# ChicyChen/LOCO-Edit

Measured on AMD Instinct MI355X. Metric: edit-directions/sec (top-5 PMP-Jacobian SVD @256^2) + vT cos-sim vs ref, higher is better.
Workload: dtype bf16x3 (split-bf16 MFMA operands, fp32 accumulate + fp32 storage); 1 GPU; CelebA-HQ DDPM 256x256 top-5 local basis (l_eye-sized mask, L=2400), t=0.6T, 12 power iterations, one GPU; multi_gpu_form=single, probes_total=5, probes_per_gpu=5, kept=5, n_iter=12, mask_L=2400, weights=synthetic seed 0, streams=2

## Files before the change

loco-edit_amd/csrc/conv_bf16_kernel.h:

```cpp
#pragma once
#include "kernels.h"
#include <cstdlib>
#include <type_traits>

namespace loco {


typedef float f32x16 __attribute__((ext_vector_type(16)));
typedef float f32x4 __attribute__((ext_vector_type(4)));
typedef f32x4 f32x4_u __attribute__((aligned(4)));
typedef float f32x2 __attribute__((ext_vector_type(2)));
typedef f32x2 f32x2_u __attribute__((aligned(4)));
typedef __bf16 bf16x8 __attribute__((ext_vector_type(8)));
typedef _Float16 f16x8 __attribute__((ext_vector_type(8)));
typedef short s16x8 __attribute__((ext_vector_type(8)));

enum : int { PR_BF16X3 = 0, PR_F16 = 1 };

constexpr int BKC = 16;
constexpr bool LIVE_MASK = true;
constexpr bool EARLY_W = true;
constexpr int NDUMMY = 8;

__device__ __forceinline__ float sigmoidf2_(float y) { return __builtin_amdgcn_rcpf(1.0f + __expf(-y)); }

__device__ __forceinline__ int idiv_small(int n, int d) {
    int q = (int)((float)n * __builtin_amdgcn_rcpf((float)d));
    const int r = n - q * d;
    q += (r >= d) ? 1 : ((r < 0) ? -1 : 0);
    return q;
}
__device__ __forceinline__ void idivmod_small(int n, int d, int& q, int& r) { q = idiv_small(n, d); r = n - q * d; }

template <int PR>
__device__ __forceinline__ int rec_off(int p, int q) {
    if constexpr (PR == PR_F16) return p * 32 + ((q ^ ((p >> 3) & 1)) << 4);
    else return p * 64 + ((q ^ ((p >> 2) & 3)) << 4);
}
template <int PR> constexpr int halo_pitch() { return PR == PR_F16 ? 48 : 80; }
template <int PR> constexpr int rec_bytes() { return PR == PR_F16 ? 32 : 64; }
template <int PR>
__device__ __forceinline__ int hrec_off(int p, int q) { return p * halo_pitch<PR>() + (q << 4); }

template <int PR>
__device__ __forceinline__ void cvt2(float a, float b, unsigned& hi, unsigned& lo) {
    if constexpr (PR == PR_F16) {
        _Float16 ha = (_Float16)a, hb = (_Float16)b;
        hi = (unsigned)__builtin_bit_cast(unsigned short, ha) | ((unsigned)__builtin_bit_cast(unsigned short, hb) << 16);
        lo = 0;
    } else {
        typedef float f32x2_ __attribute__((ext_vector_type(2)));
        typedef __bf16 bf16x2_ __attribute__((ext_vector_type(2)));
        hi = __builtin_bit_cast(unsigned, __builtin_convertvector((f32x2_){a, b}, bf16x2_));
        const float ha = __builtin_bit_cast(float, hi << 16), hb = __builtin_bit_cast(float, hi & 0xffff0000u);
// ... 387 lines not shown
                                           (fmaf(xb[0], vb[0], xb[1] * vb[1]) + fmaf(xb[2], vb[2], xb[3] * vb[3]));
            }
        }
    }
    if (tan_st) {
        constexpr int STEPS = rs_steps(NV, 64), LEFT = NV >> STEPS;
        static_assert((NV & (NV - 1)) == 0, "row sums per lane");
        rs_reduce<NV, 1, 64>(av, lane);
        if (lane < (1 << STEPS)) {
            int base = 0;
#pragma unroll
            for (int sb = 0; sb < STEPS; ++sb) base += ((lane >> sb) & 1) * (NV >> (sb + 1));
            const int ntl = (a.Hout * a.Wout) / NT, ntile = 2 * ntl;
            float* const sp = a.st_part + (long)b * C * ntile * 2;
#pragma unroll
            for (int i = 0; i < LEFT; ++i) {
                const int idx = base + i, hq = idx >> 1;
                const int h = hq / NP, q = hq - h * NP;
                const int co = ch0 + h * 32 + q * RSTEP + row0;
                sp[((long)co * ntile + pa * ntl + tile_id) * 2 + (idx & 1)] = av[i];
            }
        }
    }
}

template <int PR, int TAPS, int WM, int WN, int TM, int TN, int MODE, int STG, int PHASE = 0>
__device__ __forceinline__ void conv_lowp_body(const ConvArgs& a, f32x16 (&acc)[TM][TN]) {
    constexpr int NTHR = WM * WN * 64;
    constexpr int HP = halo_pitch<PR>();
    constexpr int RB = rec_bytes<PR>();
    constexpr int NPC = RB / 16;
    constexpr int MT = WM * TM * 32;
    constexpr int NT = WN * TN * 32;
    constexpr bool POLY = (TAPS == 4 && STG == 0), PIN = (TAPS == 4 && STG == 1);
    static_assert(TAPS != 4 || POLY || PIN, "4-tap kernels: the two polyphase forms");
    static_assert(!PIN || (MODE == CM_NONE && PHASE == 0), "polyphase input form: raw");
    constexpr int KS = (TAPS == 9) ? 3 : (TAPS == 4 ? 2 : 1);
    constexpr int HK = (TAPS == 1) ? 1 : 3;
    constexpr int NTS = KS;
    constexpr int NROW = KS;
    static_assert(!POLY || (WM == 2 && TM == 2 && MODE == CM_NONE && PHASE == 0), "polyphase output form: 128 x 256 tile, raw vector staging");
    constexpr bool NEEDP = (MODE == CM_TAN_SILU || MODE == CM_COT_SILU);
    constexpr bool GEN = (STG == 1 || STG == 2);
    constexpr int NITEM = GEN ? (2 * max_halo(NT, TAPS, STG == 2) + NTHR - 1) / NTHR : 1;
    constexpr int WTOT = NTS * MT * NPC;
    constexpr int NWV = (WTOT + NTHR - 1) / NTHR;
    constexpr bool XPF = (TAPS == 9 && STG != 2);
    constexpr int NWB = XPF ? 3 : 2;
    constexpr bool DEEP1 = (TAPS == 1 && STG == 1 && !NEEDP);
    constexpr int DEEP_D = 4;

    extern __shared__ __attribute__((aligned(16))) unsigned char smem_b[];
#ifdef LOCO_DUAL_STAMP
#define LP_STAMP(i) do { if (threadIdx.x == 0 && PHASE == 0) reinterpret_cast<unsigned long long*>(a.partial)[blockIdx.x * 8 + (i)] = __builtin_amdgcn_s_memtime(); } while (0)
#else
#define LP_STAMP(i) do { } while (0)
#endif
    LP_STAMP(0);
    constexpr int WBYTES = NTS * MT * RB;
    unsigned char* const Wsb = smem_b;
    unsigned char* Hsb;
    unsigned char* Ws = smem_b;
    unsigned char* Hs = smem_b;

    const int tid = threadIdx.x;
    const int lane = tid & 63;
    const int wave = tid >> 6;
    const int l31 = lane & 31;
    const int khalf = lane >> 5;
    const int wm = wave / WN, wn = wave % WN;

    const int S = a.stride;
    const int TW = (TAPS == 1 && PHASE == 0 && a.stride == 1 && !a.upsample && !a.zins && (a.Wout & (a.Wout - 1)) == 0)
                       ? (a.Wout < NT ? a.Wout : NT) : (a.Wout < 32 ? a.Wout : 32);
    const int TH = NT / TW;
    const int tiles_x = a.Wout / TW;
    int tile_id, cot_id, zid;
    {
        const int ntile = (a.Hout * a.Wout) / NT, ncot = (a.Cout + MT - 1) / MT, Z = a.B * a.nsplit;
        const int NTC = ntile * ncot, L = blockIdx.x;
        int T = 0;
// ... 65 lines not shown
    const long in_plane = PIN ? 4L * a.Hin * a.Win : (long)a.Hin * a.Win;

    int ipos[NITEM], ioct[NITEM];
    unsigned ivoff[NITEM];
    bool ival[NITEM];
#pragma unroll
    for (int i = 0; i < NITEM; ++i) {
        int it = tid + i * NTHR;
        int oct, pos;
        idivmod_small(it, halo_sz, oct, pos);
        int off = -1;
        if (it < 2 * halo_sz) {
            int hy, hx;
            idivmod_small(pos, halo_w, hy, hx);
            int Y = oy0 * S - a.pad + hy, X = ox0 * S - a.pad + hx;
            if (Y >= 0 && Y < LH && X >= 0 && X < LW) {
                if (a.upsample) off = (Y >> 1) * a.Win + (X >> 1);
                else if (a.zins) off = ((Y | X) & 1) ? -1 : (Y >> 1) * a.Win + (X >> 1);
                else off = PIN ? 4 * Y * a.Win + 2 * X : Y * a.Win + X;
            }
        } else {
            pos = -1; oct = 0;
        }
        ipos[i] = pos; ioct[i] = oct;
        ival[i] = off >= 0;
        ivoff[i] = (unsigned)(oct * 8 * (int)in_plane + (off >= 0 ? off : 0));
    }

    const int nseg = (halo_w + 3) >> 2;
    int v_q4 = 0, v_pos0 = -1, v_voff = 0, v_cnt = 0;
    unsigned v_pm = 0;
    int v_rec[4] = {0, 0, 0, 0};
    unsigned v_goff = 0;
    if constexpr (!GEN) {
        const int per_q = halo_h * nseg;
        const int nsg4 = (nseg + 3) >> 2, nhy2 = (halo_h + 1) >> 1;
        bool have = false;
        int hy = 0, sg = 0;
        if (32 * nsg4 * nhy2 <= NTHR) {
            const int hi = tid >> 5;
            v_q4 = (tid >> 3) & 3;
            int hq_, hr_;
            idivmod_small(hi, nsg4, hq_, hr_);
            sg = hr_ * 4 + (tid & 3);
            hy = hq_ * 2 + ((tid >> 2) & 1);
            have = hi < nsg4 * nhy2 && sg < nseg && hy < halo_h;
            if (!have) v_q4 = 0;
        } else if (tid < 4 * per_q) {
            int rem;
            idivmod_small(tid, per_q, v_q4, rem);
            idivmod_small(rem, nseg, hy, sg);
            have = true;
        }
        if (have) {
            int Y = oy0 - a.pad + hy, X0 = ox0 - a.pad + 4 * sg;
            bool rowok = (Y >= 0 && Y < a.Hin);
            v_pos0 = hy * halo_w + 4 * sg;
            v_cnt = halo_w - 4 * sg < 4 ? halo_w - 4 * sg : 4;
            v_voff = rowok ? Y * a.Win + X0 : 0;
#pragma unroll
            for (int pxi = 0; pxi < 4; ++pxi)
                if (rowok && X0 + pxi >= 0 && X0 + pxi < a.Win && pxi < v_cnt) v_pm |= 1u << pxi;
        }
#pragma unroll
        for (int pxi = 0; pxi < 4; ++pxi)
            v_rec[pxi] = (v_pos0 >= 0 && pxi < v_cnt) ? v_pos0 + pxi : halo_sz + (tid & (NDUMMY - 1));
        v_goff = (unsigned)(((long)v_q4 * 4 * in_plane + v_voff + 16) * 4);
// ... 342 lines not shown
#elif defined(LOCO_WI_2MFMA)
            acc[i][j] = __builtin_amdgcn_mfma_f32_32x32x16_bf16(ah, bl, acc[i][j], 0, 0, 0);
            acc[i][j] = __builtin_amdgcn_mfma_f32_32x32x16_bf16(ah, bh, acc[i][j], 0, 0, 0);
            (void)al;
            return;
#endif
            acc[i][j] = __builtin_amdgcn_mfma_f32_32x32x16_bf16(al, bh, acc[i][j], 0, 0, 0);
            acc[i][j] = __builtin_amdgcn_mfma_f32_32x32x16_bf16(ah, bl, acc[i][j], 0, 0, 0);
            acc[i][j] = __builtin_amdgcn_mfma_f32_32x32x16_bf16(ah, bh, acc[i][j], 0, 0, 0);
        }
    };
    auto mma_frag_head = [&](const Frag& f) { mma_one(f, 0, 0); };
    auto mma_frag_tail = [&](const Frag& f) {
#pragma unroll
        for (int i = 0; i < TM; ++i)
#pragma unroll
            for (int j = 0; j < TN; ++j)
                if (i + j > 0) mma_one(f, i, j);
    };

    const int nch = cend - cbeg;
    const int clast = cend - 1;
    auto cclamp = [&](int c) { return __builtin_amdgcn_readfirstlane(c < clast ? c : clast); };
    auto vres = [&](int x) -> int {
        if (x <= clast) { pf_live = true; return __builtin_amdgcn_readfirstlane(x); }
        pf_live = !LIVE_MASK;
        return clast;
    };
    auto stage_end = [&]() {
        asm volatile("s_waitcnt lgkmcnt(0)" ::: "memory");
        __builtin_amdgcn_s_barrier();
        asm volatile("" ::: "memory");
    };
    if constexpr (XPF) {
        Frag fr[2];
        auto stage_of = [&](int ci_, int row_, int& c_out, int& r_out) {
            c_out = cclamp(cbeg + ci_ + row_ / NROW);
            r_out = row_ % NROW;
        };
        LP_STAMP(1);
        if (nch > 0) {
            if constexpr (!(PHASE != 2 && EARLY_W)) {
                int c1, r1;
                dma_w(cbeg, 0, Wsb);
                stage_of(0, 1, c1, r1);
                dma_w(c1, r1, Wsb + WBYTES);
            }
            Hs = Hsb;
            if constexpr (!GEN && NPART == 2) {
                HaloRegs hr2;
                prefetch_hv(hr, cbeg, 0);
                prefetch_hv(hr2, cbeg, 1);
                stage_hv(hr, 0);
                stage_hv(hr2, 1);
            } else {
                prefetch_h(cbeg, 0);
                stage_h(cbeg, 0);
            }
            asm volatile("s_waitcnt vmcnt(0)" ::: "memory");
            prefetch_h(cclamp(cbeg + 1), 0);
            stage_end();
            Ws = Wsb; Hs = Hsb;
            load_frag(fr[0], 0, 0);
        }
        LP_STAMP(2);
        auto chunk_body = [&](auto ptag, const int ci) {
            constexpr int P = decltype(ptag)::value;
// ... 222 lines not shown
constexpr int lowp_min_waves(int taps, int nthr) { return (taps == 1 && nthr <= 256) ? 2 : 1; }
template <int TAPS, int WM, int WN, int TM, int TN, int MODE, int STG>
__global__ __launch_bounds__(WM * WN * 64, lowp_min_waves(TAPS, WM * WN * 64)) void conv_mfma_bf16x3(ConvArgs a) {
    f32x16 acc[TM][TN];
    conv_lowp_body<PR_BF16X3, TAPS, WM, WN, TM, TN, MODE, STG>(a, acc);
}
template <int TAPS, int WM, int WN, int TM, int TN, int MODE, int STG>
__global__ __launch_bounds__(WM * WN * 64, lowp_min_waves(TAPS, WM * WN * 64)) void conv_mfma_f16(ConvArgs a) {
    f32x16 acc[TM][TN];
    conv_lowp_body<PR_F16, TAPS, WM, WN, TM, TN, MODE, STG>(a, acc);
}

template <int PR, int WM, int WN, int TM, int TN, int MODE>
__device__ __forceinline__ void conv_lowp_kcat(const ConvArgs& a) {
    f32x16 acc[TM][TN];
    conv_lowp_body<PR, 9, WM, WN, TM, TN, MODE, 0, 1>(a, acc);
    ConvArgs a2 = a;
    a2.in = a.in2; a2.in_bs = a.in2_bs; a2.Cin = a.Cin2; a2.wb = a.wb2; a2.mode = CM_NONE; a2.pad = 0; a2.in_padded = a.in2_padded;
    conv_lowp_body<PR, 1, WM, WN, TM, TN, CM_NONE, 1, 2>(a2, acc);
}
template <int WM, int WN, int TM, int TN, int MODE>
__global__ __launch_bounds__(WM * WN * 64) void conv_kcat_bf16x3(ConvArgs a) { conv_lowp_kcat<PR_BF16X3, WM, WN, TM, TN, MODE>(a); }
template <int WM, int WN, int TM, int TN, int MODE>
__global__ __launch_bounds__(WM * WN * 64) void conv_kcat_f16(ConvArgs a) { conv_lowp_kcat<PR_F16, WM, WN, TM, TN, MODE>(a); }

template <int PR, int TAPS, int WM, int WN, int TM, int TN, int MODE, int STG>
static void launch_one_b2(const ConvArgs& a, hipStream_t st) {
    constexpr int MT = WM * TM * 32, NT = WN * TN * 32;
    constexpr int KS = (TAPS == 9) ? 3 : (TAPS == 4 ? 2 : 1), HK = (TAPS == 1) ? 1 : 3;
    int TW = a.Wout < 32 ? a.Wout : 32;
    int TH = NT / TW;
    int halo_w = (TW - 1) * a.stride + HK, halo_h = (TH - 1) * a.stride + HK;
    const int nwb = (TAPS == 9 && STG != 2) ? 3 : 2;
    size_t lds = (size_t)nwb * KS * MT * rec_bytes<PR>() + 2 * ((size_t)halo_w * halo_h + NDUMMY) * halo_pitch<PR>();
    const size_t stage_bytes = (size_t)WM * 32 * NT * 4;
    if (lds < stage_bytes) lds = stage_bytes;
    dim3 grid(((a.Hout * a.Wout) / NT) * ((a.Cout + MT - 1) / MT) * a.B * a.nsplit);
    void (*kern)(ConvArgs);
    if constexpr (PR == PR_F16) kern = &conv_mfma_f16<TAPS, WM, WN, TM, TN, MODE, STG>;
    else kern = &conv_mfma_bf16x3<TAPS, WM, WN, TM, TN, MODE, STG>;
    if (lds > 64 * 1024) {
        static DeviceOnce once;
        if (first_on_device(once)) {
            (void)hipFuncSetAttribute(reinterpret_cast<const void*>(kern), hipFuncAttributeMaxDynamicSharedMemorySize,
                                      160 * 1024);
        }
    }
    hipLaunchKernelGGL(kern, grid, dim3(WM * WN * 64), lds, st, a);
}

template <int PR, int TAPS, int WM, int WN, int TM, int TN, int MODE>
static void launch_one_b(const ConvArgs& a, hipStream_t st) {
    const bool general = a.stride != 1 || a.upsample || a.zins || (a.Cin % BKC) != 0 || !a.in_padded;
    if constexpr (MODE == CM_NONE) {
        if (a.stride == 2) launch_one_b2<PR, TAPS, WM, WN, TM, TN, MODE, 2>(a, st);
        else if (TAPS == 9 && !general) launch_one_b2<PR, TAPS, WM, WN, TM, TN, MODE, 0>(a, st);
        else launch_one_b2<PR, TAPS, WM, WN, TM, TN, MODE, 1>(a, st);
        return;
    }
    if constexpr (MODE == CM_GN_SILU || MODE == CM_TAN_SILU || MODE == CM_GN_GELU) {
        if (general) { launch_one_b2<PR, TAPS, WM, WN, TM, TN, MODE, 1>(a, st); return; }
    }
    launch_one_b2<PR, TAPS, WM, WN, TM, TN, MODE, 0>(a, st);
}


template <int PR, int MODE>
void launch_kcat_b(const ConvArgs& a, hipStream_t st) {
    constexpr int WM = 2, WN = 4, TM = 2, TN = 2, MT = 128, NT = 256;
    const int TW = a.Wout < 32 ? a.Wout : 32, TH = NT / TW;
    size_t lds = (size_t)3 * 3 * MT * rec_bytes<PR>() + 2 * ((size_t)(TW + 2) * (TH + 2) + NDUMMY) * halo_pitch<PR>();
    dim3 grid(((a.Hout * a.Wout) / NT) * ((a.Cout + MT - 1) / MT) * a.B * a.nsplit);
    void (*kern)(ConvArgs);
    if constexpr (PR == PR_F16) kern = &conv_kcat_f16<WM, WN, TM, TN, MODE>;
    else kern = &conv_kcat_bf16x3<WM, WN, TM, TN, MODE>;
    static DeviceOnce once;
    if (first_on_device(once))
        (void)hipFuncSetAttribute(reinterpret_cast<const void*>(kern), hipFuncAttributeMaxDynamicSharedMemorySize, 160 * 1024);
    hipLaunchKernelGGL(kern, grid, dim3(WM * WN * 64), lds, st, a);
}

template <int PR>
void launch_poly_b(const ConvArgs& a, hipStream_t st) {
    ConvArgs v = a;
    v.Cout = 4 * a.Cout; v.Hout = a.Hin; v.Wout = a.Win;
    v.upsample = 0; v.zins = 0; v.stride = 1; v.pad = 1; v.nsplit = 1;
    launch_one_b2<PR, 4, 2, 4, 2, 2, CM_NONE, 0>(v, st);
}

template <int PR>
void launch_poly_in_b(const ConvArgs& a, hipStream_t st) {
    ConvArgs v = a;
    v.Cin = 4 * a.Cin; v.Hin = a.Hin / 2; v.Win = a.Win / 2;
    v.upsample = 0; v.zins = 0; v.stride = 1; v.pad = 1; v.nsplit = 1;
    launch_one_b2<PR, 4, 2, 4, 2, 2, CM_NONE, 1>(v, st);
}

template <int PR, int TAPS, int MODE>
void launch_tile_b(const ConvArgs& a, hipStream_t st) {
    switch (a.tile) {
        case 5:
            launch_one_b<PR, TAPS, 2, 4, 2, 2, MODE>(a, st);
            break;
        case 0: launch_one_b<PR, TAPS, 2, 2, 2, 2, MODE>(a, st); break;
        case 1: launch_one_b<PR, TAPS, 4, 1, 1, 2, MODE>(a, st); break;
        case 2: launch_one_b<PR, TAPS, 1, 4, 1, 1, MODE>(a, st); break;
        default: launch_one_b<PR, TAPS, 2, 2, 1, 1, MODE>(a, st); break;
    }
}


}
```

loco-edit_amd/csrc/conv_plan.hip:

```cpp
#include "kernels.h"
#include <cstdio>
#include <cstdlib>

namespace loco {

constexpr int BKC = 16;
constexpr int BKF = 8;

static const int kMT[6] = {128, 128, 32, 64, 128, 128}, kNT[6] = {128, 64, 128, 64, 256, 256};

static int env_int(const char* name, int dflt) {
    const char* e = getenv(name);
    return e ? atoi(e) : dflt;
}
static int pick_tile(int Cout, int HW) {
    if (HW >= 128) return Cout > 32 ? 0 : 2;
    return Cout > 64 ? 1 : 3;
}

static int conv_pick_nsplit(int Cin, int Cout, int Hout, int Wout, int B) {
    const int t = pick_tile(Cout, Hout * Wout);
    long blocks = (long)((Hout * Wout) / kNT[t]) * ((Cout + kMT[t] - 1) / kMT[t]) * B;
    int nchunks = (Cin + BKF - 1) / BKF;
    if (blocks >= 384 || nchunks < 8) return 1;
// ... 15 lines not shown
}

constexpr int kTile0MaxHW = 65536;

static int bf16_tile_of(const ConvArgs& a, int tile_override = -1) {
    int tile = conv_bf16_pick_tile(a.Cout, a.Hout * a.Wout, a.B, tile_override);
    if (tile == 4) tile = 5;
    if (tile == 5 && a.taps == 1 && !a.gemm && a.B >= 2 && a.Hout * a.Wout <= kTile0MaxHW) return 0;
    if (a.stride == 2 && tile == 5) tile = 0;
    return tile;
}
static int tile_for(const ConvArgs& a, int prec, int tile_override) {
    return prec ? bf16_tile_of(a, tile_override) : pick_tile(a.Cout, a.Hout * a.Wout);
}
static int conv_bf16_tile_pixels(const ConvArgs& a) { return a.poly == 1 ? 512 : a.gemm ? 256 : kNT[a.tile]; }
int conv_bf16_tile_couts(const ConvArgs& a) { return a.gemm ? 64 * a.gemm_tm : kMT[a.tile]; }

static bool conv_poly_ok(const ConvEnv& e, const ConvArgs& a, int taps) {
    static const bool on = env_int("LOCO_POLYPHASE", 1) != 0;
    if (!on || e.prec < 1 || taps != 9 || a.mode != CM_NONE || !(a.upsample || a.zins) || a.stride != 1) return false;
    if (!(e.prec == 2 ? a.wph : a.wpb) || !a.in_padded || a.res || a.Cin2 > 0 || a.cot_d) return false;
    if (a.upsample ? a.pad != 1 : (a.pad != 1 && a.pad != 2)) return false;
    if ((a.Cin % BKC) != 0 || (a.Cout % 128) != 0 || a.B < 2) return false;
    if (a.Hin * a.Win < 4096 || a.Win < 32 || (a.Win % 32) != 0 || (a.Hin % 8) != 0) return false;
    return a.Hout == 2 * a.Hin && a.Wout == 2 * a.Win;
}
static bool conv_poly_in_ok(const ConvEnv& e, const ConvArgs& a, int taps) {
    static const bool on = env_int("LOCO_POLYPHASE", 1) != 0;
    if (!on || e.prec < 1 || taps != 9 || a.mode != CM_NONE || !a.pool2 || a.upsample || a.zins || a.stride != 1 || a.pad != 1) return false;
    if (!(e.prec == 2 ? a.wqh : a.wqb) || a.res || a.bias2 || a.Cin2 > 0 || a.cot_d) return false;
    if ((a.Cin % BKC) != 0 || (a.Cout % 128) != 0 || a.B < 2 || ((a.Hin | a.Win) & 1)) return false;
    if (a.Hout * a.Wout < 4096 || a.Wout < 32 || (a.Wout % 32) != 0 || (a.Hout % 8) != 0) return false;
    return a.Hin == 2 * a.Hout && a.Win == 2 * a.Wout;
}

static int conv_bf16_pick_nsplit(int Cin, int Cout, int Hout, int Wout, int B, int chip_share, int taps, int lanes) {
    const int HW = Hout * Wout;
    int t = conv_bf16_pick_tile(Cout, HW, B, -1);
    if (t == 4) t = 5;
    if (taps == 1 && t == 5 && B >= 2 && HW <= kTile0MaxHW) t = 0;
    long blocks = (long)(HW / kNT[t]) * ((Cout + kMT[t] - 1) / kMT[t]) * B;
    int nchunks = (Cin + BKC - 1) / BKC;
    int target = chip_share > 1 ? 256 / chip_share : (lanes == 2 ? 240 : 256);
    if (target < 32) target = 32;
    if (blocks >= target / 2 || nchunks < 8) return 1;
    int want = (int)(target / blocks);
    int maxs = nchunks / 4;
    if (want > maxs) want = maxs;
    if (want > 32) want = 32;
    return want < 1 ? 1 : want;
}

static bool conv_lowp_can_kcat(const ConvArgs& a) {
    static const bool on = env_int("LOCO_KCAT", 1) != 0;
    return on && a.Cin2 > 0 && a.nsplit == 1 && bf16_tile_of(a) == 5 && a.stride == 1 && !a.upsample && !a.zins && a.pad == 1 &&
           (a.Cin % BKC) == 0 && (a.Cin2 % BKC) == 0 && a.in_padded &&
           (a.mode == CM_GN_SILU || a.mode == CM_GN_GELU || a.mode == CM_TAN_SILU);
}
static bool conv_lowp_can_fuse_stats(const ConvArgs& a) {
    return a.nsplit <= 1 && !a.gemm && (a.Cout % conv_bf16_tile_couts(a)) == 0;
}

static bool conv_pair_ok(const ConvArgs& a) {
    static const bool on = env_int("LOCO_CONV_PAIR", 1) != 0;
    if (!on || a.poly || a.Hout * a.Wout < 16384 || a.taps != 9 || a.Cin2 > 0 || a.nsplit != 1 || a.stride != 1 || a.upsample || a.zins ||
        a.pad != 1 || !a.in_padded || (a.Cin % (2 * BKC)) != 0 || (a.Cout % 128) != 0 || (a.Wout % 32) != 0 || (a.Hout % 8) != 0)
// ... 92 lines not shown
        return epi;
    }
    const bool cot_cache = q->kind == ST_COT && q->norm && q->sx && x.poly != 1;
    if ((q->kind == ST_TAN || cot_cache) && e.fuse_lin && !x.cot_d && conv_lowp_can_fuse_stats(x)) {
        const size_t lane_off = (size_t)e.lane_s0 * (q->keep_floats / e.max_batch);
        const bool keptl = q->kind == ST_TAN && q->keep && s0 == 0 && x.B == B && lane_off + need <= q->keep_floats;
        if (keptl || (q->norm && need <= e.stpart_floats)) {
            x.st_part = keptl ? q->keep + lane_off : e.stpart; x.st_kind = q->kind; x.st_x = q->prim;
            if (q->kind == ST_COT) x.st_sx = q->sx;
            if (keptl) *keep_ntile = ntile;
            return epi;
        }
    }
    return alone;
}

static ConvLaunch plan_launch(const ConvEnv& e, const StatAsk* q, bool want, const ConvArgs& x, int s0, int B, int* keep_ntile) {
    ConvLaunch l;
    l.args = x;
    l.s0 = s0;
    l.args.tile = tile_for(x, e.prec, -1);
    l.stats = stats_route(e, q, want, l.args, s0, B, keep_ntile);
    if (l.stats == SR_EPI || l.stats == SR_KEEP) l.ntile = (x.Hout * x.Wout) / conv_bf16_tile_pixels(l.args);
    conv_plan_tile_pair(l.args, e.prec, -1);
    return l;
}

ConvPlan plan_conv(const ConvEnv& e, const ConvArgs& a0, int taps, const StatAsk* q, const ConvArgs* sc) {
    ConvPlan p;
    ConvArgs a = a0;
    a.taps = taps;
    a.gemm = 0;
    a.poly = 0;
    if (a.pool2) {
        if (conv_poly_in_ok(e, a, taps)) a.poly = 2;
        else {
            p.pool_after = true; p.pool_out = a.out; p.pool_out_bs = a.out_bs; p.pool_acc = a.accumulate;
            a.out = a.pool_tmp; a.out_bs = a.pool_tmp_bs; a.Hout = a.Hin; a.Wout = a.Win; a.accumulate = 0; a.pool2 = 0;
        }
    }
    if (sc) {
        ConvArgs t = a;
        t.nsplit = e.prec >= 1 ? conv_bf16_pick_nsplit(a.Cin, a.Cout, a.Hout, a.Wout, a.B, e.chip_share, 9, e.lanes) : 2;
        t.in2 = sc->in; t.in2_bs = sc->in_bs; t.Cin2 = sc->Cin;
        const long per_probe = (long)((a.Hout * a.Wout) / 256) * ((a.Cout + 127) / 128);
        if (e.prec >= 1 && taps == 9 && !short_tail(per_probe, a.B) && !a.bias2 && conv_lowp_can_kcat(t)) {
            a.in2 = sc->in; a.in2_bs = sc->in_bs; a.Cin2 = sc->Cin; a.in2_padded = sc->in_padded;
            a.wb2 = e.prec == 2 ? sc->wh : sc->wb;
            a.bias2 = sc->bias; a.bias2_bs = 0;
            a.res = nullptr;
        } else {
            p.sc_first = true;
            a.res = sc->out; a.res_bs = sc->out_bs;
        }
    }
    if (e.prec == 2) a.wb = a.wh;
    a.no_deep = e.deep1 ? 0 : 1;
    a.nsplit = e.prec >= 1 ? conv_bf16_pick_nsplit(a.Cin, a.Cout, a.Hout, a.Wout, a.B, e.chip_share, taps, e.lanes)
                           : conv_pick_nsplit(a.Cin, a.Cout, a.Hout, a.Wout, a.B);
    if (a.cot_d) {
        ConvArgs t = a;
        t.tile = bf16_tile_of(t);
        const long per_probe = (long)((a.Hout * a.Wout) / conv_bf16_tile_pixels(t)) * ((a.Cout + 127) / 128);
        p.cot = e.prec >= 1 && taps == 1 && a.nsplit == 1 && !short_tail(per_probe, a.B) && conv_lowp_can_fuse_stats(t);
        if (!p.cot) { a.cot_d = nullptr; a.cot_d_bs = 0; a.cot_sx = nullptr; a.cot_tc = nullptr; a.cot_tc_bs = 0; }
    }
    while (a.nsplit > 1 && (size_t)a.nsplit * a.B * a.Cout * a.Hout * a.Wout > e.partial_floats) a.nsplit >>= 1;
    if (a.nsplit < 1) a.nsplit = 1;
// ... 99 lines not shown
```

loco-edit_amd/csrc/engine_diag.hip:

```cpp
#include <cmath>
#include <cstdio>
#include <cstdlib>
#include <cstring>
#include <initializer_list>

#include "../../include/loco_hip_diag.h"
#include "conv_plan_text.h"
#include "engine_internal.h"

using namespace loco;
using namespace loco::eng;

static void release_since(loco_ctx* c, hipStream_t st, size_t owned0, size_t bytes0) {
    (void)hipStreamSynchronize(st);
    while (c->owned.size() > owned0) { (void)hipFree(c->owned.back()); c->owned.pop_back(); }
    c->bytes = bytes0;
}

__global__ void diag_fill_records(unsigned char* rec, long nrec, int wpitch, unsigned seed, float scale) {
    const long r = (long)blockIdx.x * 256 + threadIdx.x;
    if (r >= nrec) return;
    const int idx = (int)(r % wpitch);
    unsigned short hi[16], lo[16];
    for (int k = 0; k < 16; ++k) {
// ... 49 lines not shown
    a.prim = c->arenaP; a.prim_bs = 0; a.sx = c->sxcache;
    a.w = wf; a.wb = wf; a.wh = wf;
    a.out = out; a.out_bs = out_e; a.Cout = cout; a.Hout = H; a.Wout = W; a.B = B;
    a.mode = mode; a.pad = taps == 9 ? 1 : 0; a.in_padded = 1; a.taps = taps;
    if (geom == 4) {
        a.pool2 = 1; a.pool_tmp = out; a.pool_tmp_bs = out_e;
        a.out = out + out_e * B; a.out_bs = out_e / 4; a.Hout = H / 2; a.Wout = W / 2;
        a.wqb = wf; a.wqh = wf;
    } else if (geom) {
        a.Hin = H / 2; a.Win = W / 2;
        if (geom == 1) a.upsample = 1; else { a.zins = 1; a.pad = geom == 2 ? 2 : 1; }
        a.wpb = wf; a.wph = wf;
    }
    a.sc = c->statsP; a.sh = c->statsP + cin; a.scsh_bs = 0; a.mr = c->statsP + 2 * cin; a.mr_bs = 0;
    a.gamma_ = c->statsP; a.tst = c->statsT; a.tst_bs = c->prog->stats_per_sample; a.cpg = cin / c->cfg.gn_groups;
    a.tc = c->statsT + 64; a.tc_bs = c->prog->stats_per_sample;
    if (a.cpg < 1) a.cpg = 1;
    a.nsplit = 1; a.partial = c->partial;
    a.partial_floats = c->partial_floats - wfl * 2;
    if (getenv("LOCO_BENCH_COT") && atoi(getenv("LOCO_BENCH_COT")) && taps == 1) {
        if ((in_e + 2 * out_e) * B > (long)c->cfg.max_batch * c->prog->per_sample || out_e > c->prog->sx_total ||
            2L * cout > c->prog->stats_per_sample) { c->err = "bench_conv: cot operands exceed the arenas"; return -2; }
        launch_fill_random(out + out_e * B, out_e * B, 8u, zs, st);
        if (out_e > in_e) launch_fill_random(reinterpret_cast<float*>(c->sxcache), 2 * out_e, 3u, zs, st);
        a.cot_d = out + out_e * B; a.cot_d_bs = out_e; a.cot_sx = c->sxcache; a.cot_tc = c->statsT; a.cot_tc_bs = c->prog->stats_per_sample;
    }
    if (getenv("LOCO_BENCH_ACC") && atoi(getenv("LOCO_BENCH_ACC"))) a.accumulate = 1;
    conv_plan_family(a, c->prec);
    if (const char* e = getenv("LOCO_DUAL_WHATIF")) a.no_deep = atoi(e);
    conv_plan_tile_pair(a, c->prec, tile);
    if (geom) {
        ConvEnv e;
        e.prec = c->prec; e.partial = a.partial; e.partial_floats = a.partial_floats; e.max_batch = c->cfg.max_batch;
        a.poly = plan_conv(e, a, taps, nullptr, nullptr).l[0].args.poly;
        if (a.poly) a.nsplit = 1;
        if (geom == 4 && a.poly != 2) { c->err = "bench_conv: the shape does not take the pooled polyphase launch"; return -2; }
    }
    auto run = [&]() {
        if (c->prec == 1) launch_conv_bf16x3(a, taps, st);
        else if (c->prec == 2) launch_conv_f16(a, taps, st);
        else launch_conv(a, taps, st);
        launch_conv_splitk_reduce(a, st);
    };
    run();
    HIPCHK(c, hipEventRecord(c->ev0, st));
    for (int i = 0; i < iters; ++i) run();
    HIPCHK(c, hipEventRecord(c->ev1, st));
    HIPCHK(c, hipEventSynchronize(c->ev1));
    c->bench_out = out; c->bench_out_count = (int64_t)out_e * B;
    float ms = 0.f;
    HIPCHK(c, hipEventElapsedTime(&ms, c->ev0, c->ev1));
    *ms_avg = ms / iters;
    HIPCHK(c, hipGetLastError());
    return 0;
}

}
__global__ void diag_scale_tc(const float* tc, const float* mr, int C, int cpg, long n, int by_rstd, float* out) {
    const long i = (long)blockIdx.x * 256 + threadIdx.x;
    if (i >= n) return;
    const float f = by_rstd ? mr[2 * (int)((i % C) / cpg) + 1] : 1.0f;
    out[2 * i] = f * tc[2 * i];
    out[2 * i + 1] = f * tc[2 * i + 1];
}
extern "C" {
int loco_debug_conv(loco_ctx* c, const loco_conv_desc* d, char* plan, int64_t cap, void* stream) {
    if (!c) return -2;
// ... 619 lines not shown
```

loco-edit_amd/csrc/kernels.h:

```cpp
#pragma once
#include <hip/hip_runtime.h>
#include <stdint.h>

namespace loco {

struct DeviceOnce { bool seen[64] = {}; };
inline bool first_on_device(DeviceOnce& f) {
    int d = 0;
    (void)hipGetDevice(&d);
    d &= 63;
    if (f.seen[d]) return false;
    f.seen[d] = true;
    return true;
}


enum ConvMode : int {
    CM_NONE = 0,
    CM_GN_SILU = 1,
    CM_GN = 2,
    CM_TAN_SILU = 3,
    CM_COT_SILU = 4,
    CM_GN_GELU = 5,
};
// ... 23 lines not shown
    const float* res; long res_bs;
    const float* sc; const float* sh; long scsh_bs;
    const float* mr; long mr_bs;
    const float* gamma_;
    const float* tst; long tst_bs;
    const float* tc; long tc_bs;
    int cpg;
    int mode;
    int stride;
    int pad;
    int upsample;
    int zins;
    int in_padded;
    int accumulate;
    int nsplit;
    int taps;
    int no_deep;
    float* partial;
    int B;
    float* st_part; int st_kind;
    const float* st_x; const float2* st_sx;
    const float* in2; long in2_bs; int Cin2; int in2_padded;
    const void* wb2;
    const float* cot_d; long cot_d_bs; const float2* cot_sx; const float* cot_tc; long cot_tc_bs;
    int act;
    float res_scale;
    int gemm, gemm_tm;
    size_t partial_floats;
    int tile, pair;
    const void* wpb; const void* wph;
    int poly;
    int pool2; float* pool_tmp; long pool_tmp_bs;
    const void* wqb; const void* wqh;
};

enum PolyKind : int { POLY_UP = 0, POLY_ZINS_PAD2 = 1, POLY_ZINS_PAD1 = 2 };
inline int polyphase_vcout(int C, int a, int b, int co) { return ((a * (C / 64) + co / 64) * 2 + b) * 64 + (co % 64); }
void polyphase_fold(int kind, int nin, int nout, const float* w, long so, long si, long st, float* out);
void polyphase_fold_in(int nin, int nout, const float* w, long so, long si, long st, float* out, int noutP);

void launch_conv(const ConvArgs& a, int taps, hipStream_t st);
void launch_conv_bf16x3(const ConvArgs& a, int taps, hipStream_t st);
void launch_conv_f16(const ConvArgs& a, int taps, hipStream_t st);
void launch_conv_splitk_reduce(const ConvArgs& a, hipStream_t st);

struct ConvEnv {
    int prec = 1;
    int chip_share = 1;
    int lanes = 1, lane_s0 = 0;
    float* partial = nullptr; size_t partial_floats = 0;
    float* stpart = nullptr; size_t stpart_floats = 0;
    bool fuse_stats = true, fuse_lin = true, deep1 = true;
    int max_batch = 1;
};

struct StatAsk {
    int kind = ST_NONE;
    bool norm = false;
    const float2* sx = nullptr;
    const float* prim = nullptr;
    float* keep = nullptr; size_t keep_floats = 0;
};

enum StatRoute : int {
    SR_NONE = 0,
    SR_EPI = 1,
// ... 220 lines not shown
```

Measured before the change: 20.65 edit-directions/s.

## Add row-staged vectorized polyphase input conv path with deeper halo buffering

Adds a new staging form (STG==3) for the pooled polyphase-input 4-tap conv. Each thread loads contiguous float4 runs of the padded full-resolution input, covering two row parities, and splits them into bf16 hi/lo halo records for both column phases. It uses four halo buffers so the next channel pair's halo stores overlap the current MMAs. The aim is fewer scattered gather loads and better overlap of loads with compute. In exchange it uses more LDS, which may cut occupancy, and it only runs when the input is padded.

```diff
diff --git a/loco-edit_amd/csrc/conv_bf16_kernel.h b/loco-edit_amd/csrc/conv_bf16_kernel.h
--- a/loco-edit_amd/csrc/conv_bf16_kernel.h
+++ b/loco-edit_amd/csrc/conv_bf16_kernel.h
@@ -1,5 +1,6 @@
 #pragma once
 #include "kernels.h"
+#include "poly_in_vec.h"
 #include <cstdlib>
 #include <type_traits>
 
@@ -20,6 +21,11 @@
 constexpr int BKC = 16;
 constexpr bool LIVE_MASK = true;
 constexpr bool EARLY_W = true;
+#ifndef LOCO_PIV_NHB
+#define LOCO_PIV_NHB 4
+#endif
+constexpr int PIV_NHB = LOCO_PIV_NHB;
+static_assert(PIV_NHB == 4 || PIV_NHB == 2, "halo buffers of the row-staged polyphase input form");
 constexpr int NDUMMY = 8;
 
 __device__ __forceinline__ float sigmoidf2_(float y) { return __builtin_amdgcn_rcpf(1.0f + __expf(-y)); }
@@ -473,7 +479,7 @@
     constexpr int NPC = RB / 16;
     constexpr int MT = WM * TM * 32;
     constexpr int NT = WN * TN * 32;
-    constexpr bool POLY = (TAPS == 4 && STG == 0), PIN = (TAPS == 4 && STG == 1);
+    constexpr bool POLY = (TAPS == 4 && STG == 0), PIN = (TAPS == 4 && (STG == 1 || STG == 3)), PINV = (TAPS == 4 && STG == 3);
     static_assert(TAPS != 4 || POLY || PIN, "4-tap kernels: the two polyphase forms");
     static_assert(!PIN || (MODE == CM_NONE && PHASE == 0), "polyphase input form: raw");
     constexpr int KS = (TAPS == 9) ? 3 : (TAPS == 4 ? 2 : 1);
@@ -488,6 +494,7 @@
     constexpr int NWV = (WTOT + NTHR - 1) / NTHR;
     constexpr bool XPF = (TAPS == 9 && STG != 2);
     constexpr int NWB = XPF ? 3 : 2;
+    constexpr int NHB = PINV ? PIV_NHB : 2;
     constexpr bool DEEP1 = (TAPS == 1 && STG == 1 && !NEEDP);
     constexpr int DEEP_D = 4;
 
@@ -619,7 +626,7 @@
     unsigned v_pm = 0;
     int v_rec[4] = {0, 0, 0, 0};
     unsigned v_goff = 0;
-    if constexpr (!GEN) {
+    if constexpr (!GEN && !PINV) {
         const int per_q = halo_h * nseg;
         const int nsg4 = (nseg + 3) >> 2, nhy2 = (halo_h + 1) >> 1;
         bool have = false;
@@ -1028,7 +1035,93 @@
         __builtin_amdgcn_s_barrier();
         asm volatile("" ::: "memory");
     };
-    if constexpr (XPF) {
+    if constexpr (PINV) {
+        const int cpp = a.Cin >> 6;
+        const int npair = 2 * cpp;
+        const int H2 = 2 * a.Hin, W2 = 2 * a.Win;
+        const bool have = tid < PIV_ITEMS;
+        const PolyInVecItem it0 = poly_in_vec_item(have ? tid : 0, oy0, ox0, 0, H2, W2);
+        const PolyInVecItem it1 = poly_in_vec_item(have ? tid : 0, oy0, ox0, 1, H2, W2);
+        const int p_oct = have ? it0.oct : ((tid >> 3) & 1);
+        const unsigned obase = have ? (unsigned)(it0.oct * 8) * (unsigned)in_plane : 0u;
+        const unsigned gob0 = (obase + (have ? it0.goff : 0u)) * 4u, gob1 = (obase + (have ? it1.goff : 0u)) * 4u;
+        const bool gin0 = have && it0.inside, gin1 = have && it1.inside;
+        int p_rec[2];
+#pragma unroll
+        for (int h = 0; h < 2; ++h) p_rec[h] = (have && it0.rec[h] >= 0) ? it0.rec[h] : halo_sz + (tid & (NDUMMY - 1));
+        f32x4 dq[8];
+        const long pb4 = in_plane * 4;
+        auto wchunk = [&](int pi, int q) { return __builtin_amdgcn_readfirstlane(poly_in_vec_wchunk(pi, q, cpp)); };
+        auto piv_load = [&](int pi) {
+            const bool live = LIVE_MASK ? (pi < npair) : true;
+            const int pc = pi < npair ? pi : npair - 1;
+            const int p = pc >= cpp ? 1 : 0, c = pc - p * cpp;
+            const unsigned go = (p ? gob1 : gob0) & (live ? 0xffffffffu : 0u);
+            const unsigned char* pk = reinterpret_cast<const unsigned char*>(inb) + (long)(c * BKC) * pb4;
+#pragma unroll
+            for (int k = 0; k < 8; ++k) {
+                dq[k] = *reinterpret_cast<const f32x4_u*>(pk + go);
+                pk += pb4;
+            }
+        };
+        auto piv_store = [&](int q, bool inside, unsigned char* Hd) {
+#pragma unroll
+            for (int h = 0; h < 2; ++h) {
+                float v[8];
+#pragma unroll
+                for (int k = 0; k < 8; ++k) v[k] = inside ? dq[k][2 * h + q] : 0.0f;
+                uint4 hi, lo;
+                split8<PR>(v, hi, lo);
+                *reinterpret_cast<uint4*>(Hd + hrec_off<PR>(p_rec[h], p_oct)) = hi;
+                if constexpr (PR == PR_BF16X3) *reinterpret_cast<uint4*>(Hd + hrec_off<PR>(p_rec[h], 2 + p_oct)) = lo;
+            }
+        };
+        dma_w(wchunk(0, 0), 0, Wsb);
+        piv_load(0);
+        piv_store(0, gin0, Hsb);
+        piv_store(1, gin0, Hsb + HBYTES);
+        asm volatile("s_waitcnt vmcnt(0)" ::: "memory");
+        stage_end();
+        for (int pi = 0; pi < npair; ++pi) {
+            const int p = pi >= cpp ? 1 : 0;
+            const bool gin_n = (pi + 1 >= cpp) ? gin1 : gin0;
+            unsigned char* const Hc = NHB == 4 ? Hsb + (pi & 1) * (2 * HBYTES) : Hsb;
+            unsigned char* const Hn = Hsb + ((pi + 1) & 1) * (2 * HBYTES);
+#pragma unroll
+            for (int s = 0; s < 4; ++s) {
+                const int q = s >> 1, row = s & 1;
+                unsigned char* const Wcur = Wsb + (s & 1) * WBYTES;
+                unsigned char* const Wnxt = Wsb + ((s + 1) & 1) * WBYTES;
+                if (s < 3) {
+                    dma_w(wchunk(pi, (s + 1) >> 1), (s + 1) & 1, Wnxt);
+                } else {
+                    dma_live = LIVE_MASK ? (pi + 1 < npair) : true;
+                    dma_w(wchunk(pi + 1 < npair ? pi + 1 : pi, 0), 0, Wnxt);
+                    dma_live = true;
+                }
+                Ws = Wcur; Hs = Hc + q * HBYTES;
+                tap0 = (1 - p) * halo_w + 1 - q;
+                Frag f0, f1;
+                load_frag(f0, row, 0);
+                load_frag(f1, row, 1);
+                __builtin_amdgcn_sched_barrier(0);
+                mma_frag(f0);
+                __builtin_amdgcn_sched_barrier(0);
+                if (s == 0) piv_load(pi + 1);
+                mma_frag(f1);
+                if (NHB == 4 && s >= 2) piv_store(s - 2, gin_n, Hn + (s - 2) * HBYTES);
+                __builtin_amdgcn_sched_barrier(0);
+                if (s == 0) asm volatile("s_waitcnt vmcnt(8)" ::: "memory");
+                else asm volatile("s_waitcnt vmcnt(0)" ::: "memory");
+                stage_end();
+            }
+            if constexpr (NHB == 2) {
+                piv_store(0, gin_n, Hsb);
+                piv_store(1, gin_n, Hsb + HBYTES);
+                stage_end();
+            }
+        }
+    } else if constexpr (XPF) {
         Frag fr[2];
         auto stage_of = [&](int ci_, int row_, int& c_out, int& r_out) {
             c_out = cclamp(cbeg + ci_ + row_ / NROW);
@@ -1317,7 +1410,8 @@
     int TH = NT / TW;
     int halo_w = (TW - 1) * a.stride + HK, halo_h = (TH - 1) * a.stride + HK;
     const int nwb = (TAPS == 9 && STG != 2) ? 3 : 2;
-    size_t lds = (size_t)nwb * KS * MT * rec_bytes<PR>() + 2 * ((size_t)halo_w * halo_h + NDUMMY) * halo_pitch<PR>();
+    const int nhb = (TAPS == 4 && STG == 3) ? PIV_NHB : 2;
+    size_t lds = (size_t)nwb * KS * MT * rec_bytes<PR>() + nhb * ((size_t)halo_w * halo_h + NDUMMY) * halo_pitch<PR>();
     const size_t stage_bytes = (size_t)WM * 32 * NT * 4;
     if (lds < stage_bytes) lds = stage_bytes;
     dim3 grid(((a.Hout * a.Wout) / NT) * ((a.Cout + MT - 1) / MT) * a.B * a.nsplit);
@@ -1378,7 +1472,8 @@
     ConvArgs v = a;
     v.Cin = 4 * a.Cin; v.Hin = a.Hin / 2; v.Win = a.Win / 2;
     v.upsample = 0; v.zins = 0; v.stride = 1; v.pad = 1; v.nsplit = 1;
-    launch_one_b2<PR, 4, 2, 4, 2, 2, CM_NONE, 1>(v, st);
+    if (a.poly_vec) launch_one_b2<PR, 4, 2, 4, 2, 2, CM_NONE, 3>(v, st);
+    else launch_one_b2<PR, 4, 2, 4, 2, 2, CM_NONE, 1>(v, st);
 }
 
 template <int PR, int TAPS, int MODE>
diff --git a/loco-edit_amd/csrc/conv_plan.hip b/loco-edit_amd/csrc/conv_plan.hip
--- a/loco-edit_amd/csrc/conv_plan.hip
+++ b/loco-edit_amd/csrc/conv_plan.hip
@@ -71,6 +71,10 @@
     if ((a.Cin % BKC) != 0 || (a.Cout % 128) != 0 || a.B < 2 || ((a.Hin | a.Win) & 1)) return false;
     if (a.Hout * a.Wout < 4096 || a.Wout < 32 || (a.Wout % 32) != 0 || (a.Hout % 8) != 0) return false;
     return a.Hin == 2 * a.Hout && a.Win == 2 * a.Wout;
+}
+static bool conv_poly_in_vec_ok(const ConvArgs& a) {
+    static const bool on = env_int("LOCO_POLY_IN_VEC", 1) != 0;
+    return on && a.in_padded != 0;
 }
 
 static int conv_bf16_pick_nsplit(int Cin, int Cout, int Hout, int Wout, int B, int chip_share, int taps, int lanes) {
@@ -229,8 +233,9 @@
     a.taps = taps;
     a.gemm = 0;
     a.poly = 0;
+    a.poly_vec = 0;
     if (a.pool2) {
-        if (conv_poly_in_ok(e, a, taps)) a.poly = 2;
+        if (conv_poly_in_ok(e, a, taps)) { a.poly = 2; a.poly_vec = conv_poly_in_vec_ok(a) ? 1 : 0; }
         else {
             p.pool_after = true; p.pool_out = a.out; p.pool_out_bs = a.out_bs; p.pool_acc = a.accumulate;
             a.out = a.pool_tmp; a.out_bs = a.pool_tmp_bs; a.Hout = a.Hin; a.Wout = a.Win; a.accumulate = 0; a.pool2 = 0;
diff --git a/loco-edit_amd/csrc/engine_diag.hip b/loco-edit_amd/csrc/engine_diag.hip
--- a/loco-edit_amd/csrc/engine_diag.hip
+++ b/loco-edit_amd/csrc/engine_diag.hip
@@ -105,7 +105,8 @@
     if (geom) {
         ConvEnv e;
         e.prec = c->prec; e.partial = a.partial; e.partial_floats = a.partial_floats; e.max_batch = c->cfg.max_batch;
-        a.poly = plan_conv(e, a, taps, nullptr, nullptr).l[0].args.poly;
+        const ConvArgs planned = plan_conv(e, a, taps, nullptr, nullptr).l[0].args;
+        a.poly = planned.poly; a.poly_vec = planned.poly_vec;
         if (a.poly) a.nsplit = 1;
         if (geom == 4 && a.poly != 2) { c->err = "bench_conv: the shape does not take the pooled polyphase launch"; return -2; }
     }
diff --git a/loco-edit_amd/csrc/kernels.h b/loco-edit_amd/csrc/kernels.h
--- a/loco-edit_amd/csrc/kernels.h
+++ b/loco-edit_amd/csrc/kernels.h
@@ -79,6 +79,7 @@
     int poly;
     int pool2; float* pool_tmp; long pool_tmp_bs;
     const void* wqb; const void* wqh;
+    int poly_vec;
 };
 
 enum PolyKind : int { POLY_UP = 0, POLY_ZINS_PAD2 = 1, POLY_ZINS_PAD1 = 2 };
diff --git a/loco-edit_amd/csrc/poly_in_vec.h b/loco-edit_amd/csrc/poly_in_vec.h
--- /dev/null
+++ b/loco-edit_amd/csrc/poly_in_vec.h
@@ -0,0 +1,41 @@
+#pragma once
+
+#if !defined(__host__) && !defined(__HIPCC__)
+#define __host__
+#define __device__
+#endif
+
+namespace loco {
+
+constexpr int PIV_TW = 32, PIV_TH = 8;
+constexpr int PIV_HW = PIV_TW + 2, PIV_HH = PIV_TH + 2;
+constexpr int PIV_NV = (2 * PIV_HW + 4) / 4;
+constexpr int PIV_ITEMS = 2 * PIV_HH * PIV_NV;
+
+struct PolyInVecItem {
+    int oct;
+    unsigned goff;
+    int inside;
+    int rec[2];
+};
+
+__host__ __device__ inline PolyInVecItem poly_in_vec_item(int it, int oy0, int ox0, int p, int H2, int W2) {
+    PolyInVecItem r;
+    const int j = it % PIV_NV, t = it / PIV_NV;
+    const int hy = t % PIV_HH;
+    r.oct = t / PIV_HH;
+    const int R = 2 * (oy0 - 1 + hy) + p, C0 = 2 * ox0 - 4 + 4 * j;
+    r.inside = (R >= 0 && R < H2 && C0 >= 0 && C0 + 3 < W2) ? 1 : 0;
+    r.goff = r.inside ? (unsigned)(R * W2 + C0) : 0u;
+    const int hx0 = 2 * j - 1, hx1 = 2 * j;
+    r.rec[0] = hx0 >= 0 ? hy * PIV_HW + hx0 : -1;
+    r.rec[1] = hx1 < PIV_HW ? hy * PIV_HW + hx1 : -1;
+    return r;
+}
+
+__host__ __device__ inline int poly_in_vec_wchunk(int pi, int q, int cpp) {
+    const int p = pi >= cpp ? 1 : 0;
+    return (2 * p + q) * cpp + (pi - p * cpp);
+}
+
+}
```

Measured after the change: 20.75 edit-directions/s, median of 6. About the same (+0.5%).
